# atakan-topaloglu/stable-virtual-camera

Hardware: AMD Instinct MI355X
Metric: denoising steps/sec, 1.3B Seva @ 21x576x576 views (higher is better)
Workload: dtype f16; 1 GPU; Seva 1.3B (1,263,968,004 params, random-init), one 21-view window per GPU, 576x576 px (latent 72x72), CFG batch 42, Euler-EDM step, MultiviewCFG(1.2) cfg 2.0; novel_views_per_sec = value x (T - 1 input view) / 50 steps per window; views=21, latent=72, windows=1

## Files before the change

stable-virtual-camera_amd/csrc/capi.hip:

```cpp
#include "seva_common.h"

#include <stdarg.h>
#include <stdio.h>
#include <stdlib.h>
#include <string.h>

#include <mutex>
#include <vector>

namespace {

thread_local char g_err[512] = "";

struct ProfRecord {
  int cls;
  double work, bytes;
  hipEvent_t e0, e1;
};
std::mutex g_prof_mu;
std::vector<ProfRecord> g_prof;
bool g_prof_on = false;

}

namespace {
struct KnobEntry {
  const char* name;
  const char* env;
  int SevaKnobs::*field;
};
const KnobEntry kKnobs[] = {
    {"gemm_chunks", "SEVA_GEMM_CHUNKS", &SevaKnobs::gemm_chunks}, {"gemm_dbg", "SEVA_GEMM_DBG", &SevaKnobs::gemm_dbg},
    {"gemm_stagger", "SEVA_GEMM_STAGGER", &SevaKnobs::gemm_stagger},
    {"gemm_bm", "SEVA_GEMM_BM", &SevaKnobs::gemm_bm}, {"gemm_bn", "SEVA_GEMM_BN", &SevaKnobs::gemm_bn},
    {"gemm_astat", "SEVA_GEMM_ASTAT", &SevaKnobs::gemm_astat}, {"attn_dbg", "SEVA_ATTN_DBG", &SevaKnobs::attn_dbg},
    {"attn_no_tr", "SEVA_ATTN_NO_TR", &SevaKnobs::attn_no_tr}, {"attn_two", "SEVA_ATTN_TWO", &SevaKnobs::attn_two},
    {"attn_split", "SEVA_ATTN_SPLIT", &SevaKnobs::attn_split},
    {"gn_min_iter", "SEVA_GN_MIN_ITER", &SevaKnobs::gn_min_iter},
    {"conv_win", "SEVA_CONV_WIN", &SevaKnobs::conv_win},
};
SevaKnobs knobs_from_env() {
  SevaKnobs k;
  for (const auto& e : kKnobs) {
    const char* v = getenv(e.env);
    k.*(e.field) = (v && v[0]) ? atoi(v) : -1;
  }
  return k;
}
}

SevaKnobs g_seva_knobs = knobs_from_env();

thread_local const char* g_seva_last_plan = "";

void seva_set_error(const char* fmt, ...) {
  va_list ap;
  va_start(ap, fmt);
  vsnprintf(g_err, sizeof(g_err), fmt, ap);
  va_end(ap);
}

int seva_check_launch(const char* what) {
  hipError_t e = hipGetLastError();
  if (e != hipSuccess) {
    seva_set_error("%s: launch failed: %s", what, hipGetErrorString(e));
    return SEVA_ERR_LAUNCH;
  }
  return SEVA_OK;
}

SevaProfScope::SevaProfScope(int cls_, double work_, hipStream_t stream_, double bytes_)
    : cls(cls_), work(work_), bytes(bytes_ < 0 ? work_ : bytes_), stream(stream_), e0(nullptr), e1(nullptr), on(g_prof_on) {
  if (!on) return;
  if (hipEventCreate(&e0) != hipSuccess || hipEventCreate(&e1) != hipSuccess) {
    on = false;
    return;
  }
  (void)hipEventRecord(e0, stream);
}

SevaProfScope::~SevaProfScope() {
  if (!on) return;
  (void)hipEventRecord(e1, stream);
  std::lock_guard<std::mutex> lk(g_prof_mu);
  g_prof.push_back({cls, work, bytes, e0, e1});
}

extern "C" {

const char* seva_last_error(void) { return g_err; }
const char* seva_last_plan(void) { return g_seva_last_plan; }
int seva_abi_version(void) { return 12; }
const char* seva_target_arch(void) { return "gfx950"; }

int seva_set_knob(const char* name, int value) {
  SEVA_REQUIRE(name != nullptr, "set_knob: null name");
  for (const auto& e : kKnobs)
    if (strcmp(e.name, name) == 0) {
      g_seva_knobs.*(e.field) = value;
      return SEVA_OK;
    }
  seva_set_error("set_knob: unknown knob '%s'", name);
  return SEVA_ERR_ARG;
}

int seva_get_knob(const char* name, int* value) {
  SEVA_REQUIRE(name != nullptr && value != nullptr, "get_knob: null argument");
  for (const auto& e : kKnobs)
    if (strcmp(e.name, name) == 0) {
      *value = g_seva_knobs.*(e.field);
      return SEVA_OK;
    }
  seva_set_error("get_knob: unknown knob '%s'", name);
  return SEVA_ERR_ARG;
}

int seva_graph_begin(seva_stream_t stream) {
  hipError_t e = hipStreamBeginCapture((hipStream_t)stream, hipStreamCaptureModeThreadLocal);
  if (e != hipSuccess) {
    seva_set_error("graph_begin: %s", hipGetErrorString(e));
    return SEVA_ERR_LAUNCH;
  }
  return SEVA_OK;
}

int seva_graph_end(seva_stream_t stream, void** graph_exec_out) {
  SEVA_REQUIRE(graph_exec_out != nullptr, "graph_end: null out");
  hipGraph_t graph = nullptr;
  hipError_t e = hipStreamEndCapture((hipStream_t)stream, &graph);
  if (e != hipSuccess || graph == nullptr) {
    seva_set_error("graph_end: %s", hipGetErrorString(e));
    return SEVA_ERR_LAUNCH;
  }
  hipGraphExec_t exec = nullptr;
  e = hipGraphInstantiate(&exec, graph, nullptr, nullptr, 0);
  (void)hipGraphDestroy(graph);
  if (e != hipSuccess) {
    seva_set_error("graph_instantiate: %s", hipGetErrorString(e));
    return SEVA_ERR_LAUNCH;
  }
  *graph_exec_out = (void*)exec;
  return SEVA_OK;
}

int seva_graph_launch(void* graph_exec, seva_stream_t stream) {
  SEVA_REQUIRE(graph_exec != nullptr, "graph_launch: null graph");
  hipError_t e = hipGraphLaunch((hipGraphExec_t)graph_exec, (hipStream_t)stream);
  if (e != hipSuccess) {
    seva_set_error("graph_launch: %s", hipGetErrorString(e));
    return SEVA_ERR_LAUNCH;
  }
  return SEVA_OK;
}

int seva_graph_destroy(void* graph_exec) {
  if (graph_exec) (void)hipGraphExecDestroy((hipGraphExec_t)graph_exec);
  return SEVA_OK;
}

int seva_prof_enable(int on) {
  std::lock_guard<std::mutex> lk(g_prof_mu);
  g_prof_on = on != 0;
  return SEVA_OK;
}

int seva_prof_collect(double* ms, int64_t* launches, double* work, double* bytes) {
  SEVA_REQUIRE(ms && launches && work && bytes, "prof_collect: null out");
  hipError_t e = hipDeviceSynchronize();
  if (e != hipSuccess) {
    seva_set_error("prof_collect: %s", hipGetErrorString(e));
    return SEVA_ERR_LAUNCH;
  }
  std::lock_guard<std::mutex> lk(g_prof_mu);
  for (int i = 0; i < SEVA_PROF_CLASSES; ++i) {
    ms[i] = 0.0;
    launches[i] = 0;
    work[i] = 0.0;
    bytes[i] = 0.0;
  }
  for (auto& r : g_prof) {
    float t = 0.f;
    if (hipEventElapsedTime(&t, r.e0, r.e1) == hipSuccess && r.cls >= 0 && r.cls < SEVA_PROF_CLASSES) {
      ms[r.cls] += t;
      launches[r.cls] += 1;
      work[r.cls] += r.work;
      bytes[r.cls] += r.bytes;
    }
    (void)hipEventDestroy(r.e0);
    (void)hipEventDestroy(r.e1);
  }
  g_prof.clear();
  return SEVA_OK;
}

}
```

stable-virtual-camera_amd/csrc/ff_fused.hip:

```cpp
#include "gemm_common.h"
#include "ff_fp8.h"

#include <atomic>

namespace {

struct FfArgs {
  const half_t* a;
  const half_t* w1;
  const float* b1;
  const half_t* w2;
  const float* b2;
  const float* residual;
  float* out_f32;
  half_t* out_f16;
  int64_t M, lda, ldr, ldo32, ldo16;
  int32_t tiles_m;
  const float* ln_x;
  const float* ln_gamma;
  const float* ln_beta;
  int64_t ldx;
  float ln_eps;
};

struct Ff8Args {
  FfArgs f;
  const uint8_t* w1_exp;
  const uint8_t* w2_exp;
};

template <int N>
__device__ __forceinline__ void ff_wait_vm() {
  asm volatile("s_waitcnt vmcnt(%0)" ::"n"(N) : "memory");
}

static __device__ __forceinline__ void glds16_sv(const void* sbase, unsigned voff, unsigned lds_wave_base) {
  unsigned keep;
  asm volatile(
      "s_mov_b32 %0, m0\n\ts_mov_b32 m0, %3\n\ts_nop 0\n\tglobal_load_lds_dwordx4 %1, %2\n\ts_mov_b32 m0, %0"
      : "=&s"(keep)
      : "v"(voff), "s"(sbase), "s"(lds_wave_base)
      : "memory");
}


template <int C>
__global__ __launch_bounds__(512, 2) void ff_fused8_kernel(FfArgs p) {
  constexpr int KS = C / 32, NK1 = C / 64, NJ2 = C / 16, NJH = NJ2 / 2, NCH = C / 16;
  constexpr int W1_BYTES = 128 * 128, W2_BYTES = C * 128;
  constexpr int W2_PASSES = C / 64;
  constexpr int W2_PER_KT = (W2_PASSES + NK1 - 1) / NK1;
  static_assert(NJ2 % 2 == 0, "output blocks split over the two waves of a row group");

  extern __shared__ __attribute__((aligned(16))) char smem[];
  constexpr int W1_RING = 3;
  char* const lds_w1 = smem;
  char* const lds_w2 = smem + W1_RING * W1_BYTES;
  float* const lds_b1 = (float*)(smem + W1_RING * W1_BYTES + 2 * W2_BYTES);
  char* const lds_x = smem + W1_RING * W1_BYTES + 2 * W2_BYTES + 8 * C * 4;
  const unsigned lds_base_u32 = __builtin_amdgcn_readfirstlane(lds_addr_u32(smem));

  const int lane = threadIdx.x & 63;
  const int wave = __builtin_amdgcn_readfirstlane(threadIdx.x >> 6);
  const int mr = wave & 3, h = wave >> 2;
  const int fr = lane & 15, fg = lane >> 4;
  const int sr = lane >> 3, sp = lane & 7;

  const int tm = xcd_remap(blockIdx.x, p.tiles_m);
  const int64_t m0 = (int64_t)tm * 128 + mr * 32;

  half8_t areg[2][KS];
  if (p.ln_x) {
#pragma unroll
    for (int i = 0; i < 2; ++i) {
      int64_t m = m0 + 16 * i + fr;
      if (m >= p.M) m = p.M - 1;
      const float* xr = p.ln_x + m * p.ldx + 8 * fg;
      f32x4 v[KS][2];
#pragma unroll
      for (int ks = 0; ks < KS; ++ks) {
        v[ks][0] = first_read(*(const f32x4*)(xr + 32 * ks));
        v[ks][1] = first_read(*(const f32x4*)(xr + 32 * ks + 4));
      }
      float sum = 0.f;
#pragma unroll
      for (int ks = 0; ks < KS; ++ks)
#pragma unroll
        for (int e = 0; e < 2; ++e) sum += v[ks][e][0] + v[ks][e][1] + v[ks][e][2] + v[ks][e][3];
      sum += __shfl_xor(sum, 16, 64);
      asm volatile("" : "+v"(sum));
      sum += __shfl_xor(sum, 32, 64);
      asm volatile("" : "+v"(sum));
      const float mean = sum / (float)C;
      float ss = 0.f;
#pragma unroll
      for (int ks = 0; ks < KS; ++ks)
#pragma unroll
        for (int e = 0; e < 2; ++e)
#pragma unroll
          for (int r = 0; r < 4; ++r) {
            const float dlt = v[ks][e][r] - mean;
            ss += dlt * dlt;
          }
      ss += __shfl_xor(ss, 16, 64);
      asm volatile("" : "+v"(ss));
      ss += __shfl_xor(ss, 32, 64);
      asm volatile("" : "+v"(ss));
      const float rstd = rsqrtf(ss / (float)C + p.ln_eps);
#pragma unroll
      for (int ks = 0; ks < KS; ++ks) {
        half_t y[8];
#pragma unroll
        for (int e = 0; e < 2; ++e) {
          const f32x4 g4 = first_read(*(const f32x4*)(p.ln_gamma + 32 * ks + 8 * fg + 4 * e));
          const f32x4 b4 = first_read(*(const f32x4*)(p.ln_beta + 32 * ks + 8 * fg + 4 * e));
#pragma unroll
          for (int r = 0; r < 4; ++r) y[4 * e + r] = (half_t)((v[ks][e][r] - mean) * rstd * g4[r] + b4[r]);
        }
        areg[i][ks] = half8_t{y[0], y[1], y[2], y[3], y[4], y[5], y[6], y[7]};
      }
    }
  } else {
#pragma unroll
    for (int i = 0; i < 2; ++i) {
      int64_t m = m0 + 16 * i + fr;
      if (m >= p.M) m = p.M - 1;
      const half_t* ap = p.a + m * p.lda + 8 * fg;
#pragma unroll
      for (int ks = 0; ks < KS; ++ks) areg[i][ks] = *(const half8_t*)(ap + 32 * ks);
    }
  }
  f32x4 acc2[2][NJH];
#pragma unroll
  for (int i = 0; i < 2; ++i) {
    int64_t m = m0 + 16 * i + fr;
    if (m >= p.M) m = p.M - 1;
#pragma unroll
    for (int jj = 0; jj < NJH; ++jj)
      acc2[i][jj] = p.residual ? *(const f32x4*)(p.residual + m * p.ldr + 16 * (h * NJH + jj) + 4 * fg) : f32x4{0.f, 0.f, 0.f, 0.f};
  }
  for (int i = threadIdx.x; i < 2 * C; i += 512) *(f32x4*)(lds_b1 + 4 * i) = *(const f32x4*)(p.b1 + 4 * i);
#pragma unroll
  for (int i = 0; i < 2; ++i) {
#pragma unroll
    for (int ks = 0; ks < KS; ++ks) asm volatile("" : "+v"(areg[i][ks]));
#pragma unroll
    for (int jj = 0; jj < NJH; ++jj) asm volatile("" : "+v"(acc2[i][jj]));
  }

  auto w1_key = [](int row) { return ((row >> 1) & 1) | (((row >> 3) & 3) << 1); };
  const half_t* w1_src[2];
#pragma unroll
  for (int i = 0; i < 2; ++i) {
    const int row = wave * 16 + 8 * i + sr;
    w1_src[i] = p.w1 + (int64_t)row * C + (sp ^ w1_key(row)) * 8;
  }
  const half_t* w2_src[2];
#pragma unroll
  for (int i = 0; i < 2; ++i) {
    const int row = wave * (C / 8) + 8 * i + sr;
    w2_src[i] = p.w2 + (int64_t)row * (4 * C) + (sp ^ ((row >> 1) & 7)) * 8;
  }
  auto stage_w1 = [&](int buf, int hc, int kt) {
    const unsigned dst = lds_base_u32 + buf * W1_BYTES + wave * 16 * 128;
    const int64_t off = (int64_t)hc * 128 * C + kt * 64;
#pragma unroll
    for (int i = 0; i < 2; ++i) glds16_raw(w1_src[i] + off, dst + i * 1024);
  };
  auto stage_w2_part = [&](int buf, int hc, int part) {
    const unsigned dst = lds_base_u32 + W1_RING * W1_BYTES + buf * W2_BYTES + wave * (C / 8) * 128;
#pragma unroll
    for (int u = 0; u < W2_PER_KT; ++u) {
      const int i = part * W2_PER_KT + u;
      if (i < W2_PASSES) glds16_raw(w2_src[i & 1] + (int64_t)(i >> 1) * 16 * (4 * C) + hc * 64, dst + i * 1024);
    }
  };
  auto barrier_raw = [&]() {
    asm volatile("s_waitcnt lgkmcnt(0)" ::: "memory");
    __builtin_amdgcn_s_barrier();
    asm volatile("" ::: "memory");
  };

  int w1_off[2], w2_off[2];
#pragma unroll
  for (int s = 0; s < 2; ++s) {
    const int rb = 64 * h + 8 * (fr >> 2) + (fr & 3);
    w1_off[s] = rb * 128 + (((4 * s + fg) ^ w1_key(rb)) << 4);
    const int r2 = 16 * (h * NJH) + fr;
    w2_off[s] = r2 * 128 + (((4 * s + fg) ^ ((r2 >> 1) & 7)) << 4);
  }
  char* const x_mine = lds_x + ((mr * 2 + h) * 2) * 1024 + lane * 16;
  const char* const x_q0 = lds_x + (mr * 2 * 2) * 1024 + lane * 16;

  constexpr int NTILES = NCH * NK1;
  auto stage_w1_seq = [&](int g) { stage_w1(g % W1_RING, g / NK1, g % NK1); };
  auto wait_all_but = [&](int n) {
    if (n >= 3) ff_wait_vm<3>();
    else if (n == 2) ff_wait_vm<2>();
    else if (n == 1) ff_wait_vm<1>();
    else ff_wait_vm<0>();
  };
  __syncthreads();
  stage_w1_seq(0);
#pragma unroll
  for (int part = 0; part < NK1; ++part) stage_w2_part(0, 0, part);
  if (NTILES > 1) stage_w1_seq(1);
  if (NTILES > 1) ff_wait_vm<2>();
  else ff_wait_vm<0>();
  barrier_raw();

  int g = 0;
  for (int hc = 0; hc < NCH; ++hc) {
    f32x4 acc1[2][4];
#pragma unroll
    for (int e = 0; e < 2; ++e) {
      const float* bp = lds_b1 + hc * 128 + 64 * h + 8 * fg + 4 * e;
      acc1[0][e] = acc1[1][e] = *(const f32x4*)bp;
      acc1[0][2 + e] = acc1[1][2 + e] = *(const f32x4*)(bp + 32);
    }
#pragma unroll
    for (int kt = 0; kt < NK1; ++kt) {
      int issued = 0;
      if (g + 2 < NTILES) {
        stage_w1_seq(g + 2);
        issued += 2;
      }
      if (hc + 1 < NCH && kt * W2_PER_KT < W2_PASSES) {
        stage_w2_part((hc + 1) & 1, hc + 1, kt);
        issued += (kt + 1) * W2_PER_KT <= W2_PASSES ? W2_PER_KT : W2_PASSES - kt * W2_PER_KT;
      }
      const char* const tb = lds_w1 + (g % W1_RING) * W1_BYTES;
      half8_t bfr[2][4];
#pragma unroll
      for (int s = 0; s < 2; ++s)
#pragma unroll
        for (int j = 0; j < 4; ++j) bfr[s][j] = *(const half8_t*)(tb + w1_off[s] + (32 * (j >> 1) + 4 * (j & 1)) * 128);
#pragma unroll
      for (int s = 0; s < 2; ++s)
#pragma unroll
        for (int i = 0; i < 2; ++i)
#pragma unroll
          for (int j = 0; j < 4; ++j)
            acc1[i][j] = __builtin_amdgcn_mfma_f32_16x16x32_f16(bfr[s][j], areg[i][2 * kt + s], acc1[i][j], 0, 0, 0);
      wait_all_but(issued);
      barrier_raw();
      ++g;
    }
#pragma unroll
    for (int i = 0; i < 2; ++i) {
      const f32x4 o0 = geglu4(acc1[i][0], acc1[i][2]);
      const f32x4 o1 = geglu4(acc1[i][1], acc1[i][3]);
      *(half8_t*)(x_mine + i * 1024) = half8_t{(half_t)o0[0], (half_t)o0[1], (half_t)o0[2], (half_t)o0[3],
                                               (half_t)o1[0], (half_t)o1[1], (half_t)o1[2], (half_t)o1[3]};
    }
    barrier_raw();
    half8_t hq[2][2];
#pragma unroll
    for (int q = 0; q < 2; ++q)
#pragma unroll
      for (int i = 0; i < 2; ++i) hq[q][i] = *(const half8_t*)(x_q0 + (q * 2 + i) * 1024);
    const char* const t2 = lds_w2 + (hc & 1) * W2_BYTES;
#pragma unroll
    for (int jj = 0; jj < NJH; ++jj) {
      const half8_t w0 = *(const half8_t*)(t2 + w2_off[0] + jj * (16 * 128));
      const half8_t w1f = *(const half8_t*)(t2 + w2_off[1] + jj * (16 * 128));
#pragma unroll
      for (int i = 0; i < 2; ++i) {
        acc2[i][jj] = __builtin_amdgcn_mfma_f32_16x16x32_f16(w0, hq[0][i], acc2[i][jj], 0, 0, 0);
        acc2[i][jj] = __builtin_amdgcn_mfma_f32_16x16x32_f16(w1f, hq[1][i], acc2[i][jj], 0, 0, 0);
      }
    }
    barrier_raw();
  }

#pragma unroll
  for (int i = 0; i < 2; ++i) {
    const int64_t m = m0 + 16 * i + fr;
    const bool ok = m < p.M;
#pragma unroll
    for (int jj = 0; jj < NJH; ++jj) {
      const int f = 16 * (h * NJH + jj) + 4 * fg;
      const f32x4 v = acc2[i][jj] + first_read(*(const f32x4*)(p.b2 + f));
      if (!ok) continue;
      if (p.out_f32) *(f32x4*)(p.out_f32 + m * p.ldo32 + f) = v;
      if (p.out_f16) {
        const half4_t hh = {(half_t)v[0], (half_t)v[1], (half_t)v[2], (half_t)v[3]};
        *(half4_t*)(p.out_f16 + m * p.ldo16 + f) = hh;
      }
    }
  }
}


template <int C>
int ff_launch8(const FfArgs& a, hipStream_t s) {
  constexpr int lds = 3 * 128 * 128 + 2 * C * 128 + 8 * C * 4 + 16 * 1024;
  static std::atomic<uint64_t> attr_devs{0};
  int dev = 0;
  (void)hipGetDevice(&dev);
  const uint64_t bit = 1ull << (dev & 63);
  if (!(attr_devs.load(std::memory_order_relaxed) & bit)) {
    (void)hipFuncSetAttribute((const void*)ff_fused8_kernel<C>, hipFuncAttributeMaxDynamicSharedMemorySize, lds);
    attr_devs.fetch_or(bit, std::memory_order_relaxed);
  }
  hipLaunchKernelGGL((ff_fused8_kernel<C>), dim3((unsigned)a.tiles_m), dim3(512), lds, s, a);
  return seva_check_launch("ff_fused8_kernel");
}


template <int C>
__global__ __launch_bounds__(512, 2) void ff_fused8_fp8_kernel(Ff8Args q) {
  const FfArgs& p = q.f;
  constexpr int KP = FF8_KP(C), NK1 = KP / 128, NU = C / 64;
  constexpr int NJ2 = C / 16, NJH = NJ2 / 2, NCH = C / 16, NP = NCH / 2, NSC2 = (NJH + 3) / 4;
  constexpr int W1_BYTES = 128 * 128, W2_BYTES = C * 128;
  constexpr int W2_PASSES = C / 64;
  constexpr int W2_PER_KT = (W2_PASSES + 2 * NK1 - 1) / (2 * NK1);
  static_assert(NJ2 % 2 == 0 && NCH % 2 == 0, "output blocks split over two waves; chunks taken in pairs");
  static_assert(2 + W2_PER_KT <= 3, "wait_all_but counts at most 3 loads per K-tile");
  typedef int v4i_t __attribute__((ext_vector_type(4)));

  extern __shared__ __attribute__((aligned(16))) char smem[];
  constexpr int W1_RING = 3;
  char* const lds_w1 = smem;
  char* const lds_w2 = smem + W1_RING * W1_BYTES;
  float* const lds_b1 = (float*)(smem + W1_RING * W1_BYTES + 2 * W2_BYTES);
  int* const lds_s1 = (int*)(smem + W1_RING * W1_BYTES + 2 * W2_BYTES + 8 * C * 4);
  char* const lds_x = smem + W1_RING * W1_BYTES + 2 * W2_BYTES + 8 * C * 4 + NCH * 32 * 4;
  const unsigned lds_base_u32 = __builtin_amdgcn_readfirstlane(lds_addr_u32(smem));

  const int lane = threadIdx.x & 63;
  const int wave = __builtin_amdgcn_readfirstlane(threadIdx.x >> 6);
  const int mr = wave & 3, h = wave >> 2;
  const int fr = lane & 15, fg = lane >> 4;
  const int sr = lane >> 3, sp = lane & 7;

  const int tm = xcd_remap(blockIdx.x, p.tiles_m);
  const int64_t m0 = (int64_t)tm * 128 + mr * 32;

  half8_t areg[2][2 * NK1];
  if (p.ln_x) {
#pragma unroll
    for (int i = 0; i < 2; ++i) {
      int64_t m = m0 + 16 * i + fr;
      if (m >= p.M) m = p.M - 1;
      const float* xr = p.ln_x + m * p.ldx + 16 * fg;
      f32x4 v[NU][4];
#pragma unroll
      for (int u = 0; u < NU; ++u)
#pragma unroll
        for (int e = 0; e < 4; ++e) v[u][e] = first_read(*(const f32x4*)(xr + 64 * u + 4 * e));
      float sum = 0.f;
#pragma unroll
      for (int u = 0; u < NU; ++u)
#pragma unroll
        for (int e = 0; e < 4; ++e) sum += v[u][e][0] + v[u][e][1] + v[u][e][2] + v[u][e][3];
      sum += __shfl_xor(sum, 16, 64);
      asm volatile("" : "+v"(sum));
      sum += __shfl_xor(sum, 32, 64);
      asm volatile("" : "+v"(sum));
      const float mean = sum / (float)C;
      float ss = 0.f;
#pragma unroll
      for (int u = 0; u < NU; ++u)
#pragma unroll
        for (int e = 0; e < 4; ++e)
#pragma unroll
          for (int r = 0; r < 4; ++r) {
            const float dlt = v[u][e][r] - mean;
            ss += dlt * dlt;
          }
      ss += __shfl_xor(ss, 16, 64);
      asm volatile("" : "+v"(ss));
      ss += __shfl_xor(ss, 32, 64);
      asm volatile("" : "+v"(ss));
      const float rstd = rsqrtf(ss / (float)C + p.ln_eps);
#pragma unroll
      for (int u = 0; u < 2 * NK1; ++u) {
        if (u >= NU) {
          areg[i][u] = half8_t{};
          continue;
        }
        v4i_t w;
#pragma unroll
        for (int e = 0; e < 4; ++e) {
          const f32x4 g4 = first_read(*(const f32x4*)(p.ln_gamma + 64 * u + 16 * fg + 4 * e));
          const f32x4 b4 = first_read(*(const f32x4*)(p.ln_beta + 64 * u + 16 * fg + 4 * e));
          float y[4];
#pragma unroll
          for (int r = 0; r < 4; ++r) y[r] = (v[u][e][r] - mean) * rstd * g4[r] + b4[r];
          w[e] = pack_fp8x4(y[0], y[1], y[2], y[3]);
        }
        areg[i][u] = __builtin_bit_cast(half8_t, w);
      }
    }
  } else {
#pragma unroll
    for (int i = 0; i < 2; ++i) {
      int64_t m = m0 + 16 * i + fr;
      if (m >= p.M) m = p.M - 1;
      const uint8_t* ap = (const uint8_t*)p.a + m * p.lda + 16 * fg;
#pragma unroll
      for (int u = 0; u < 2 * NK1; ++u) areg[i][u] = u < NU ? *(const half8_t*)(ap + 64 * u) : half8_t{};
    }
  }
  f32x4 acc2[2][NJH];
#pragma unroll
  for (int i = 0; i < 2; ++i)
#pragma unroll
    for (int jj = 0; jj < NJH; ++jj) acc2[i][jj] = f32x4{0.f, 0.f, 0.f, 0.f};
  for (int i = threadIdx.x; i < 2 * C; i += 512) *(f32x4*)(lds_b1 + 4 * i) = *(const f32x4*)(p.b1 + 4 * i);
  for (int idx = threadIdx.x; idx < NCH * 32; idx += 512) {
    const int hc = idx >> 5, hh = (idx >> 4) & 1, f = idx & 15;
    const int rb = hc * 128 + 64 * hh + 8 * (f >> 2) + (f & 3);
    lds_s1[idx] = (int)q.w1_exp[rb] | ((int)q.w1_exp[rb + 4] << 8) | ((int)q.w1_exp[rb + 32] << 16) | ((int)q.w1_exp[rb + 36] << 24);
  }
  int wsc2[NSC2];
#pragma unroll
  for (int w = 0; w < NSC2; ++w) wsc2[w] = 0;
#pragma unroll
  for (int jj = 0; jj < NJH; ++jj) wsc2[jj >> 2] |= (int)q.w2_exp[16 * (h * NJH + jj) + fr] << (8 * (jj & 3));
#pragma unroll
  for (int i = 0; i < 2; ++i) {
#pragma unroll
    for (int u = 0; u < NU; ++u) asm volatile("" : "+v"(areg[i][u]));
#pragma unroll
    for (int jj = 0; jj < NJH; ++jj) asm volatile("" : "+v"(acc2[i][jj]));
  }
#pragma unroll
  for (int w = 0; w < NSC2; ++w) asm volatile("" : "+v"(wsc2[w]));

  auto w1_key = [](int row) { return ((row >> 1) & 1) | (((row >> 3) & 3) << 1); };
  unsigned w1_voff[2];
#pragma unroll
  for (int i = 0; i < 2; ++i) {
    const int row = wave * 16 + 8 * i + sr;
    w1_voff[i] = (unsigned)(row * KP + (sp ^ w1_key(row)) * 16);
  }
  unsigned w2_voff[2];
#pragma unroll
  for (int i = 0; i < 2; ++i) {
    const int row = wave * (C / 8) + 8 * i + sr;
    w2_voff[i] = (unsigned)(row * (4 * C) + (sp ^ ((row >> 1) & 7)) * 16);
  }
  auto stage_w1 = [&](int buf, int hc, int kt) {
    const unsigned dst = lds_base_u32 + buf * W1_BYTES + wave * 16 * 128;
    const uint8_t* const base = (const uint8_t*)p.w1 + (int64_t)hc * 128 * KP + kt * 128;
#pragma unroll
    for (int i = 0; i < 2; ++i) glds16_sv(base, w1_voff[i], dst + i * 1024);
  };
  auto stage_w2_part = [&](int buf, int pp, int part) {
    const unsigned dst = lds_base_u32 + W1_RING * W1_BYTES + buf * W2_BYTES + wave * (C / 8) * 128;
#pragma unroll
    for (int u = 0; u < W2_PER_KT; ++u) {
      const int i = part * W2_PER_KT + u;
      if (i < W2_PASSES)
        glds16_sv((const uint8_t*)p.w2 + (int64_t)(i >> 1) * 16 * (4 * C) + pp * 128, w2_voff[i & 1], dst + i * 1024);
    }
  };
  auto barrier_raw = [&]() {
    asm volatile("s_waitcnt lgkmcnt(0)" ::: "memory");
    __builtin_amdgcn_s_barrier();
    asm volatile("" ::: "memory");
  };

  int w1_off[2], w2_off[2];
#pragma unroll
  for (int s = 0; s < 2; ++s) {
    const int rb = 64 * h + 8 * (fr >> 2) + (fr & 3);
    w1_off[s] = rb * 128 + (((4 * s + fg) ^ w1_key(rb)) << 4);
    const int r2 = 16 * (h * NJH) + fr;
    w2_off[s] = r2 * 128 + (((4 * s + fg) ^ ((r2 >> 1) & 7)) << 4);
  }
  char* const x_mine = lds_x + ((mr * 2 + h) * 2) * 1024 + lane * 16;
  const char* const x_q0 = lds_x + (mr * 2 * 2) * 1024 + lane * 16;

  constexpr int NTILES = NCH * NK1;
  auto stage_w1_seq = [&](int g) { stage_w1(g % W1_RING, g / NK1, g % NK1); };
  auto wait_all_but = [&](int n) {
    if (n >= 3) ff_wait_vm<3>();
    else if (n == 2) ff_wait_vm<2>();
    else if (n == 1) ff_wait_vm<1>();
    else ff_wait_vm<0>();
  };
  __syncthreads();
  stage_w1_seq(0);
#pragma unroll
  for (int part = 0; part < 2 * NK1; ++part) stage_w2_part(0, 0, part);
  stage_w1_seq(1);
  ff_wait_vm<2>();
  barrier_raw();

  int g = 0;
  for (int pp = 0; pp < NP; ++pp) {
    v4i_t hx[2];
#pragma unroll
    for (int c = 0; c < 2; ++c) {
      const int hc = 2 * pp + c;
      f32x4 acc1[2][4];
#pragma unroll
      for (int i = 0; i < 2; ++i)
#pragma unroll
        for (int j = 0; j < 4; ++j) acc1[i][j] = f32x4{0.f, 0.f, 0.f, 0.f};
      const int sc1 = lds_s1[hc * 32 + h * 16 + fr];
#pragma unroll
      for (int kt = 0; kt < NK1; ++kt) {
        int issued = 0;
        if (g + 2 < NTILES) {
          stage_w1_seq(g + 2);
          issued += 2;
        }
        const int kk = c * NK1 + kt;
        if (pp + 1 < NP && kk * W2_PER_KT < W2_PASSES) {
          stage_w2_part((pp + 1) & 1, pp + 1, kk);
          issued += (kk + 1) * W2_PER_KT <= W2_PASSES ? W2_PER_KT : W2_PASSES - kk * W2_PER_KT;
        }
        const char* const tb = lds_w1 + (g % W1_RING) * W1_BYTES;
#pragma unroll
        for (int jp = 0; jp < 2; ++jp) {
          half8_t bfr[2][2];
#pragma unroll
          for (int s = 0; s < 2; ++s)
#pragma unroll
            for (int e = 0; e < 2; ++e) bfr[s][e] = *(const half8_t*)(tb + w1_off[s] + (32 * jp + 4 * e) * 128);
#pragma unroll
          for (int i = 0; i < 2; ++i)
#pragma unroll
            for (int e = 0; e < 2; ++e)
              acc1[i][2 * jp + e] = mfma_f8(2 * jp + e, bfr[0][e], bfr[1][e], areg[i][2 * kt], areg[i][2 * kt + 1], acc1[i][2 * jp + e], sc1);
          if (jp == 0) __builtin_amdgcn_sched_barrier(0);
        }
#pragma unroll
        for (int i = 0; i < 2; ++i)
#pragma unroll
          for (int j = 0; j < 4; ++j) asm volatile("" : "+v"(acc1[i][j]));
        wait_all_but(issued);
        barrier_raw();
        ++g;
      }
      f32x4 bias[4];
#pragma unroll
      for (int e = 0; e < 2; ++e) {
        const float* bp = lds_b1 + hc * 128 + 64 * h + 8 * fg + 4 * e;
        bias[e] = first_read(*(const f32x4*)bp);
        bias[2 + e] = first_read(*(const f32x4*)(bp + 32));
      }
#pragma unroll
      for (int i = 0; i < 2; ++i) {
        const f32x4 o0 = geglu4(acc1[i][0] + bias[0], acc1[i][2] + bias[2]);
        const f32x4 o1 = geglu4(acc1[i][1] + bias[1], acc1[i][3] + bias[3]);
        hx[i][2 * c] = pack_fp8x4(o0[0], o0[1], o0[2], o0[3]);
        hx[i][2 * c + 1] = pack_fp8x4(o1[0], o1[1], o1[2], o1[3]);
      }
    }
#pragma unroll
    for (int i = 0; i < 2; ++i) *(v4i_t*)(x_mine + i * 1024) = hx[i];
    barrier_raw();
    half8_t hq[2][2];
#pragma unroll
    for (int qq = 0; qq < 2; ++qq)
#pragma unroll
      for (int i = 0; i < 2; ++i) hq[qq][i] = *(const half8_t*)(x_q0 + (qq * 2 + i) * 1024);
    const char* const t2 = lds_w2 + (pp & 1) * W2_BYTES;
#pragma unroll
    for (int jj = 0; jj < NJH; ++jj) {
      const half8_t w0 = *(const half8_t*)(t2 + w2_off[0] + jj * (16 * 128));
      const half8_t w1f = *(const half8_t*)(t2 + w2_off[1] + jj * (16 * 128));
#pragma unroll
      for (int i = 0; i < 2; ++i) acc2[i][jj] = mfma_f8(jj, w0, w1f, hq[0][i], hq[1][i], acc2[i][jj], wsc2[jj >> 2]);
    }
#pragma unroll
    for (int i = 0; i < 2; ++i)
#pragma unroll
      for (int jj = 0; jj < NJH; ++jj) asm volatile("" : "+v"(acc2[i][jj]));
    barrier_raw();
  }

#pragma unroll
  for (int i = 0; i < 2; ++i) {
    const int64_t m = m0 + 16 * i + fr;
    const bool ok = m < p.M;
#pragma unroll
    for (int jj = 0; jj < NJH; ++jj) {
      const int f = 16 * (h * NJH + jj) + 4 * fg;
      if (!ok) continue;
      f32x4 v = acc2[i][jj] + first_read(*(const f32x4*)(p.b2 + f));
      if (p.residual) v += first_read(*(const f32x4*)(p.residual + m * p.ldr + f));
      if (p.out_f32) *(f32x4*)(p.out_f32 + m * p.ldo32 + f) = v;
      if (p.out_f16) {
        const half4_t hh = {(half_t)v[0], (half_t)v[1], (half_t)v[2], (half_t)v[3]};
        *(half4_t*)(p.out_f16 + m * p.ldo16 + f) = hh;
      }
    }
  }
}

template <int C>
int ff_launch8_fp8(const Ff8Args& a, hipStream_t s) {
  constexpr int lds = 3 * 128 * 128 + 2 * C * 128 + 8 * C * 4 + (C / 16) * 32 * 4 + 16 * 1024;
  static_assert(lds <= 160 * 1024, "LDS budget of one workgroup per CU");
  static std::atomic<uint64_t> attr_devs{0};
  int dev = 0;
  (void)hipGetDevice(&dev);
  const uint64_t bit = 1ull << (dev & 63);
  if (!(attr_devs.load(std::memory_order_relaxed) & bit)) {
    (void)hipFuncSetAttribute((const void*)ff_fused8_fp8_kernel<C>, hipFuncAttributeMaxDynamicSharedMemorySize, lds);
    attr_devs.fetch_or(bit, std::memory_order_relaxed);
  }
// ... 84 lines not shown
```

stable-virtual-camera_amd/csrc/gemm_plan_dump.cpp:

```cpp
#include <stdio.h>
#include <stdlib.h>
#include <string.h>

#include <string>

#include "gemm_plan.h"

using namespace seva_plan;

static void print_gemm_cfg(const GemmCfg& c) {
  printf("\tbm=%d\tbn=%d\tmode=%d\tepi=%d\tdbgk=%d\tpaired=%d\tastat=%d\tfp8=%d\tsplitk=%d\tnw=%d\tsplit16=%d", c.bm, c.bn, c.mode, c.epi, c.dbgk,
         c.paired, c.astat, c.fp8, c.splitk, c.nw, c.split16);
}
static void print_win_cfg(const WinCfg& c) {
  printf("\tbm=%d\tbn=%d\tnw=%d\twcap=%d\tdbw=%d\tstats=%d\tup=%d\ttw=%d\tfp8=%d\to8=%d\ts2=%d\tph=%d", c.bm, c.bn, c.nw, c.wcap, c.dbw, c.stats,
         c.up, c.tw, c.fp8, c.o8, c.s2, c.ph);
}

static int print_tables() {
  for (int i = 0; i < kNumGemmKernels; ++i) {
    printf("table=gemm\trow=%d\tname=%s\thas_dbgk=%d", i, kGemmKernels[i].name, has_dbgk(kGemmKernels[i].cfg));
    print_gemm_cfg(kGemmKernels[i].cfg);
    printf("\n");
  }
  for (int i = 0; i < kNumWinKernels; ++i) {
    printf("table=win\trow=%d\tname=%s", i, kWinKernels[i].name);
    print_win_cfg(kWinKernels[i].cfg);
    printf("\n");
  }
  return 0;
}

int main() {
  static char line[4096];
  void* const set = (void*)(uintptr_t)64;
  while (fgets(line, sizeof line, stdin)) {
    if (strncmp(line, "tables", 6) == 0) {
      print_tables();
      continue;
    }
    seva_gemm_desc d;
    memset(&d, 0, sizeof d);
    SevaKnobs k;
    k.gemm_chunks = k.gemm_dbg = k.gemm_stagger = k.gemm_bm = k.gemm_bn = k.gemm_astat = -1;
    k.attn_dbg = k.attn_no_tr = k.attn_two = k.attn_split = k.gn_min_iter = k.conv_win = -1;
    Variant v = F16;
    bool any = false, bad = false;
    for (char* tok = strtok(line, " \t\r\n"); tok; tok = strtok(nullptr, " \t\r\n")) {
      char* eq = strchr(tok, '=');
      if (!eq) { bad = true; break; }
      *eq = 0;
      const std::string key = tok, val = eq + 1;
      const long long x = atoll(val.c_str());
      any = true;
      if (key == "v") v = val == "fp8" ? FP8 : val == "split_out" ? F16_SPLIT_OUT : F16;
      else if (key == "mode") d.mode = (int)x;
      else if (key == "epi") d.epilogue = (int)x;
      else if (key == "M") d.M = x;
      else if (key == "N") d.N = x;
      else if (key == "K") d.K = x;
      else if (key == "n") d.n = (int)x;
      else if (key == "ih") d.ih = (int)x;
      else if (key == "iw") d.iw = (int)x;
      else if (key == "cin") d.cin = (int)x;
      else if (key == "oh") d.oh = (int)x;
      else if (key == "ow") d.ow = (int)x;
      else if (key == "stride") d.stride = (int)x;
      else if (key == "up") d.upsample = (int)x;
      else if (key == "pad_br") d.pad_br_only = (int)x;
      else if (key == "rpg") d.rows_per_group = x;
      else if (key == "K2") d.K2 = x;
      else if (key == "bias") d.bias = x ? (const float*)set : nullptr;
      else if (key == "row_add") d.row_add = x ? (const float*)set : nullptr;
      else if (key == "residual") d.residual = x ? (const float*)set : nullptr;
      else if (key == "out_f32") d.out_f32 = x ? (float*)set : nullptr;
      else if (key == "out_f16") d.out_f16 = x ? set : nullptr;
      else if (key == "out_f8") d.out_f8 = x ? set : nullptr;
      else if (key == "w_exp") d.w_exp = x ? set : nullptr;
      else if (key == "ch_stats") d.ch_stats = x ? (float*)set : nullptr;
      else if (key == "splitk_ws") d.splitk_ws = x ? (float*)set : nullptr;
      else if (key == "a2") d.a2 = x ? set : nullptr;
      else if (key == "gemm_bm") k.gemm_bm = (int)x;
      else if (key == "gemm_bn") k.gemm_bn = (int)x;
      else if (key == "gemm_astat") k.gemm_astat = (int)x;
      else if (key == "gemm_chunks") k.gemm_chunks = (int)x;
      else if (key == "gemm_dbg") k.gemm_dbg = (int)x;
      else if (key == "gemm_stagger") k.gemm_stagger = (int)x;
      else if (key == "conv_win") k.conv_win = (int)x;
      else { bad = true; break; }
    }
    if (!any) continue;
    if (bad) {
      printf("kernel=bad_input\n");
      continue;
    }
    d.a = set;
    d.w = set;
    const Plan p = plan(d, k, v);
    const WinPlan& w = p.window;
    static const char* const declined[] = {"none", "phases", "fp8_stride2", "fp8_window_only"};
    if (p.declined != DECLINED_NONE) {
      printf("kernel=error\tdeclined=%s", declined[p.declined]);
    } else if (p.kernel == GEMM_KERNEL) {
      const int row = find_row(p.gemm);
      printf("kernel=gemm\trow=%d\tname=%s", row, row >= 0 ? kGemmKernels[row].name : "NONE");
      print_gemm_cfg(p.gemm);
      printf("\ttiles_m=%d\ttiles_n=%d\tchunks=%d\tgrid=%lld\tdbg=%d\tstagger=%d\tsk_tiles=%lld\tsk_bn=%d", p.tiles_m, p.tiles_n, p.n_chunks,
             (long long)p.grid, p.dbg, p.stagger, (long long)p.sk_tiles, p.sk_bn);
    } else {
      const WinCfg& c = w.cand[w.win];
      const int row = find_row(c);
      printf("kernel=window\trow=%d\tname=%s", row, row >= 0 ? kWinKernels[row].name : "NONE");
      print_win_cfg(c);
      printf("\tlinear=%d\tn_lin=%d\tranges=%d\tn_full=%d\tfull=%d/%d/%d\ttail=%d/%d/%d\ttiles_n=%d", w.linear, w.geom.n_lin, w.n_ranges(), w.n_full,
             w.full.n, w.full.tpi, w.full.tiles_m, w.tail.n, w.tail.tpi, w.tail.tiles_m, w.geom.tiles_n);
      printf("\tWp=%d\tSp=%d\thw=%d\tow=%d\tmul=%u/%u/%u/%u", w.geom.Wp, w.geom.Sp, w.geom.hw, w.geom.ow, w.geom.mul_hw, w.geom.mul_iw, w.geom.mul_sp,
             w.geom.mul_wp);
    }
    printf("\twin=%d\tcands=", w.win);
    for (int i = 0; i < w.n_cand; ++i) {
      const int row = find_row(w.cand[i]);
      printf("%s%s", i ? ";" : "", row >= 0 ? kWinKernels[row].name : "NONE");
    }
    printf("\n");
  }
  return 0;
}
```

stable-virtual-camera_amd/csrc/seva_knobs.h:

```cpp
#pragma once

struct SevaKnobs {
  int gemm_chunks, gemm_dbg, gemm_stagger, gemm_bm, gemm_bn, gemm_astat;
  int attn_dbg, attn_no_tr, attn_two, attn_split;
  int gn_min_iter;
  int conv_win;
};
extern SevaKnobs g_seva_knobs;
```

Before: 11.04 denoising steps/s.

## Make fused FF kernel persistent with cross-tile weight prefetch and LDS-resident biases

Converts the fused feed-forward kernel into a persistent grid sized from an occupancy query, with each workgroup looping over M tiles. While the current tile's epilogue runs, the next tile's first W1/W2 weight tiles are already being staged. Biases b1 and b2 are loaded into LDS once per workgroup instead of once per tile, and kernel arguments are read through the kernarg pointer to ease scalar register pressure. The intent is to remove per-tile launch and prologue latency and overlap it with compute. The cost is a larger LDS footprint, a new ff_grid knob, and a risk of load imbalance when the tile count does not divide evenly across the grid.

Result: no change. 11.03 denoising steps/s (-0.1%).

```diff
diff --git a/stable-virtual-camera_amd/csrc/capi.hip b/stable-virtual-camera_amd/csrc/capi.hip
--- a/stable-virtual-camera_amd/csrc/capi.hip
+++ b/stable-virtual-camera_amd/csrc/capi.hip
@@ -37,6 +37,7 @@
     {"attn_no_tr", "SEVA_ATTN_NO_TR", &SevaKnobs::attn_no_tr}, {"attn_two", "SEVA_ATTN_TWO", &SevaKnobs::attn_two},
     {"attn_split", "SEVA_ATTN_SPLIT", &SevaKnobs::attn_split},
     {"gn_min_iter", "SEVA_GN_MIN_ITER", &SevaKnobs::gn_min_iter},
+    {"ff_grid", "SEVA_FF_GRID", &SevaKnobs::ff_grid},
     {"conv_win", "SEVA_CONV_WIN", &SevaKnobs::conv_win},
 };
 SevaKnobs knobs_from_env() {
diff --git a/stable-virtual-camera_amd/csrc/ff_fused.hip b/stable-virtual-camera_amd/csrc/ff_fused.hip
--- a/stable-virtual-camera_amd/csrc/ff_fused.hip
+++ b/stable-virtual-camera_amd/csrc/ff_fused.hip
@@ -43,6 +43,12 @@
       : "memory");
 }
 
+typedef const __attribute__((address_space(4))) FfArgs* ff_kargs_t;
+static __device__ __forceinline__ ff_kargs_t ff_kargs() {
+  ff_kargs_t q = (ff_kargs_t)__builtin_amdgcn_kernarg_segment_ptr();
+  asm volatile("" : "+s"(q));
+  return q;
+}
 
 template <int C>
 __global__ __launch_bounds__(512, 2) void ff_fused8_kernel(FfArgs p) {
@@ -58,30 +64,106 @@
   char* const lds_w2 = smem + W1_RING * W1_BYTES;
   float* const lds_b1 = (float*)(smem + W1_RING * W1_BYTES + 2 * W2_BYTES);
   char* const lds_x = smem + W1_RING * W1_BYTES + 2 * W2_BYTES + 8 * C * 4;
+  constexpr int B2_OFF = W1_RING * W1_BYTES + 2 * W2_BYTES + 8 * C * 4 + 16 * 1024;
+  const float* const lds_b2 = (const float*)(smem + B2_OFF);
   const unsigned lds_base_u32 = __builtin_amdgcn_readfirstlane(lds_addr_u32(smem));
 
   const int lane = threadIdx.x & 63;
   const int wave = __builtin_amdgcn_readfirstlane(threadIdx.x >> 6);
   const int mr = wave & 3, h = wave >> 2;
-  const int fr = lane & 15, fg = lane >> 4;
-  const int sr = lane >> 3, sp = lane & 7;
-
-  const int tm = xcd_remap(blockIdx.x, p.tiles_m);
+  for (int i = threadIdx.x; i < 2 * C; i += 512) *(f32x4*)(lds_b1 + 4 * i) = *(const f32x4*)(p.b1 + 4 * i);
+  for (int i = threadIdx.x; i < C / 4; i += 512) *(f32x4*)(smem + B2_OFF + 16 * i) = *(const f32x4*)(p.b2 + 4 * i);
+
+  auto w1_key = [](int row) { return ((row >> 1) & 1) | (((row >> 3) & 3) << 1); };
+  const half_t* w1_src[2];
+  const half_t* w2_src[2];
+  auto set_src = [&](int ln) {
+    const int sr = ln >> 3, sp = ln & 7;
+#pragma unroll
+    for (int i = 0; i < 2; ++i) {
+      const int row = wave * 16 + 8 * i + sr;
+      w1_src[i] = p.w1 + (int64_t)row * C + (sp ^ w1_key(row)) * 8;
+    }
+#pragma unroll
+    for (int i = 0; i < 2; ++i) {
+      const int row = wave * (C / 8) + 8 * i + sr;
+      w2_src[i] = p.w2 + (int64_t)row * (4 * C) + (sp ^ ((row >> 1) & 7)) * 8;
+    }
+  };
+  set_src(lane);
+  auto stage_w1 = [&](int buf, int hc, int kt) {
+    const unsigned dst = lds_base_u32 + buf * W1_BYTES + wave * 16 * 128;
+    const int64_t off = (int64_t)hc * 128 * C + kt * 64;
+#pragma unroll
+    for (int i = 0; i < 2; ++i) glds16_raw(w1_src[i] + off, dst + i * 1024);
+  };
+  auto stage_w2_part = [&](int buf, int hc, int part) {
+    const unsigned dst = lds_base_u32 + W1_RING * W1_BYTES + buf * W2_BYTES + wave * (C / 8) * 128;
+#pragma unroll
+    for (int u = 0; u < W2_PER_KT; ++u) {
+      const int i = part * W2_PER_KT + u;
+      if (i < W2_PASSES) glds16_raw(w2_src[i & 1] + (int64_t)(i >> 1) * 16 * (4 * C) + hc * 64, dst + i * 1024);
+    }
+  };
+  auto barrier_raw = [&]() {
+    asm volatile("s_waitcnt lgkmcnt(0)" ::: "memory");
+    __builtin_amdgcn_s_barrier();
+    asm volatile("" ::: "memory");
+  };
+
+  constexpr int NTILES = NCH * NK1;
+  auto stage_w1_seq = [&](int g) { stage_w1(g % W1_RING, g / NK1, g % NK1); };
+  auto stage_head = [&]() {
+    const half_t *s1a = w1_src[0], *s1b = w1_src[1], *s2a = w2_src[0], *s2b = w2_src[1];
+    unsigned lb = lds_base_u32;
+    asm volatile("" : "+v"(s1a), "+v"(s1b), "+v"(s2a), "+v"(s2b), "+s"(lb));
+    const unsigned d1 = lb + wave * 16 * 128, d2 = lb + W1_RING * W1_BYTES + wave * (C / 8) * 128;
+    glds16_raw(s1a, d1);
+    glds16_raw(s1b, d1 + 1024);
+#pragma unroll
+    for (int i = 0; i < W2_PASSES; ++i) glds16_raw(((i & 1) ? s2b : s2a) + (int64_t)(i >> 1) * 16 * (4 * C), d2 + i * 1024);
+    if (NTILES > 1) {
+      constexpr int64_t off = (int64_t)(1 / NK1) * 128 * C + (1 % NK1) * 64;
+      glds16_raw(s1a + off, d1 + W1_BYTES);
+      glds16_raw(s1b + off, d1 + W1_BYTES + 1024);
+    }
+  };
+  auto wait_all_but = [&](int n) {
+    if (n >= 3) ff_wait_vm<3>();
+    else if (n == 2) ff_wait_vm<2>();
+    else if (n == 1) ff_wait_vm<1>();
+    else ff_wait_vm<0>();
+  };
+  static_assert(2 + W2_PER_KT <= 3, "wait_all_but counts at most 3 loads per K-tile");
+
+  const int grid = (int)gridDim.x;
+  stage_head();
+  for (int vb = (int)blockIdx.x; vb < p.tiles_m; vb += grid) {
+  const int tm = xcd_remap(vb, p.tiles_m);
   const int64_t m0 = (int64_t)tm * 128 + mr * 32;
-
+  const bool more = vb + grid < p.tiles_m;
+  int lane_t = lane;
+  asm volatile("" : "+v"(lane_t));
+  const int fr = lane_t & 15, fg = lane_t >> 4;
+
+  const ff_kargs_t ph = ff_kargs();
   half8_t areg[2][KS];
-  if (p.ln_x) {
+  if (ph->ln_x) {
+    f32x4 vv[2][KS][2];
 #pragma unroll
     for (int i = 0; i < 2; ++i) {
       int64_t m = m0 + 16 * i + fr;
-      if (m >= p.M) m = p.M - 1;
-      const float* xr = p.ln_x + m * p.ldx + 8 * fg;
-      f32x4 v[KS][2];
+      if (m >= ph->M) m = ph->M - 1;
+      const float* xr = ph->ln_x + m * ph->ldx + 8 * fg;
 #pragma unroll
       for (int ks = 0; ks < KS; ++ks) {
-        v[ks][0] = first_read(*(const f32x4*)(xr + 32 * ks));
-        v[ks][1] = first_read(*(const f32x4*)(xr + 32 * ks + 4));
-      }
+        vv[i][ks][0] = first_read(*(const f32x4*)(xr + 32 * ks));
+        vv[i][ks][1] = first_read(*(const f32x4*)(xr + 32 * ks + 4));
+      }
+    }
+#pragma unroll
+    for (int i = 0; i < 2; ++i) {
+      f32x4(&v)[KS][2] = vv[i];
       float sum = 0.f;
 #pragma unroll
       for (int ks = 0; ks < KS; ++ks)
@@ -106,26 +188,27 @@
       asm volatile("" : "+v"(ss));
       ss += __shfl_xor(ss, 32, 64);
       asm volatile("" : "+v"(ss));
-      const float rstd = rsqrtf(ss / (float)C + p.ln_eps);
+      const float rstd = rsqrtf(ss / (float)C + ph->ln_eps);
 #pragma unroll
       for (int ks = 0; ks < KS; ++ks) {
         half_t y[8];
 #pragma unroll
         for (int e = 0; e < 2; ++e) {
-          const f32x4 g4 = first_read(*(const f32x4*)(p.ln_gamma + 32 * ks + 8 * fg + 4 * e));
-          const f32x4 b4 = first_read(*(const f32x4*)(p.ln_beta + 32 * ks + 8 * fg + 4 * e));
+          const f32x4 g4 = first_read(*(const f32x4*)(ph->ln_gamma + 32 * ks + 8 * fg + 4 * e));
+          const f32x4 b4 = first_read(*(const f32x4*)(ph->ln_beta + 32 * ks + 8 * fg + 4 * e));
 #pragma unroll
           for (int r = 0; r < 4; ++r) y[4 * e + r] = (half_t)((v[ks][e][r] - mean) * rstd * g4[r] + b4[r]);
         }
         areg[i][ks] = half8_t{y[0], y[1], y[2], y[3], y[4], y[5], y[6], y[7]};
       }
+      if (i == 0) __builtin_amdgcn_sched_barrier(0);
     }
   } else {
 #pragma unroll
     for (int i = 0; i < 2; ++i) {
       int64_t m = m0 + 16 * i + fr;
-      if (m >= p.M) m = p.M - 1;
-      const half_t* ap = p.a + m * p.lda + 8 * fg;
+      if (m >= ph->M) m = ph->M - 1;
+      const half_t* ap = ph->a + m * ph->lda + 8 * fg;
 #pragma unroll
       for (int ks = 0; ks < KS; ++ks) areg[i][ks] = *(const half8_t*)(ap + 32 * ks);
     }
@@ -134,12 +217,11 @@
 #pragma unroll
   for (int i = 0; i < 2; ++i) {
     int64_t m = m0 + 16 * i + fr;
-    if (m >= p.M) m = p.M - 1;
+    if (m >= ph->M) m = ph->M - 1;
 #pragma unroll
     for (int jj = 0; jj < NJH; ++jj)
-      acc2[i][jj] = p.residual ? *(const f32x4*)(p.residual + m * p.ldr + 16 * (h * NJH + jj) + 4 * fg) : f32x4{0.f, 0.f, 0.f, 0.f};
-  }
-  for (int i = threadIdx.x; i < 2 * C; i += 512) *(f32x4*)(lds_b1 + 4 * i) = *(const f32x4*)(p.b1 + 4 * i);
+      acc2[i][jj] = ph->residual ? *(const f32x4*)(ph->residual + m * ph->ldr + 16 * (h * NJH + jj) + 4 * fg) : f32x4{0.f, 0.f, 0.f, 0.f};
+  }
 #pragma unroll
   for (int i = 0; i < 2; ++i) {
 #pragma unroll
@@ -148,65 +230,22 @@
     for (int jj = 0; jj < NJH; ++jj) asm volatile("" : "+v"(acc2[i][jj]));
   }
 
-  auto w1_key = [](int row) { return ((row >> 1) & 1) | (((row >> 3) & 3) << 1); };
-  const half_t* w1_src[2];
-#pragma unroll
-  for (int i = 0; i < 2; ++i) {
-    const int row = wave * 16 + 8 * i + sr;
-    w1_src[i] = p.w1 + (int64_t)row * C + (sp ^ w1_key(row)) * 8;
-  }
-  const half_t* w2_src[2];
-#pragma unroll
-  for (int i = 0; i < 2; ++i) {
-    const int row = wave * (C / 8) + 8 * i + sr;
-    w2_src[i] = p.w2 + (int64_t)row * (4 * C) + (sp ^ ((row >> 1) & 7)) * 8;
-  }
-  auto stage_w1 = [&](int buf, int hc, int kt) {
-    const unsigned dst = lds_base_u32 + buf * W1_BYTES + wave * 16 * 128;
-    const int64_t off = (int64_t)hc * 128 * C + kt * 64;
-#pragma unroll
-    for (int i = 0; i < 2; ++i) glds16_raw(w1_src[i] + off, dst + i * 1024);
-  };
-  auto stage_w2_part = [&](int buf, int hc, int part) {
-    const unsigned dst = lds_base_u32 + W1_RING * W1_BYTES + buf * W2_BYTES + wave * (C / 8) * 128;
-#pragma unroll
-    for (int u = 0; u < W2_PER_KT; ++u) {
-      const int i = part * W2_PER_KT + u;
-      if (i < W2_PASSES) glds16_raw(w2_src[i & 1] + (int64_t)(i >> 1) * 16 * (4 * C) + hc * 64, dst + i * 1024);
-    }
-  };
-  auto barrier_raw = [&]() {
-    asm volatile("s_waitcnt lgkmcnt(0)" ::: "memory");
-    __builtin_amdgcn_s_barrier();
-    asm volatile("" ::: "memory");
-  };
-
+  int lane_c = lane;
+  asm volatile("" : "+v"(lane_c));
+  set_src(lane_c);
+  const int fr_c = lane_c & 15, fg_c = lane_c >> 4;
   int w1_off[2], w2_off[2];
 #pragma unroll
   for (int s = 0; s < 2; ++s) {
-    const int rb = 64 * h + 8 * (fr >> 2) + (fr & 3);
-    w1_off[s] = rb * 128 + (((4 * s + fg) ^ w1_key(rb)) << 4);
-    const int r2 = 16 * (h * NJH) + fr;
-    w2_off[s] = r2 * 128 + (((4 * s + fg) ^ ((r2 >> 1) & 7)) << 4);
-  }
-  char* const x_mine = lds_x + ((mr * 2 + h) * 2) * 1024 + lane * 16;
-  const char* const x_q0 = lds_x + (mr * 2 * 2) * 1024 + lane * 16;
-
-  constexpr int NTILES = NCH * NK1;
-  auto stage_w1_seq = [&](int g) { stage_w1(g % W1_RING, g / NK1, g % NK1); };
-  auto wait_all_but = [&](int n) {
-    if (n >= 3) ff_wait_vm<3>();
-    else if (n == 2) ff_wait_vm<2>();
-    else if (n == 1) ff_wait_vm<1>();
-    else ff_wait_vm<0>();
-  };
-  __syncthreads();
-  stage_w1_seq(0);
-#pragma unroll
-  for (int part = 0; part < NK1; ++part) stage_w2_part(0, 0, part);
-  if (NTILES > 1) stage_w1_seq(1);
-  if (NTILES > 1) ff_wait_vm<2>();
-  else ff_wait_vm<0>();
+    const int rb = 64 * h + 8 * (fr_c >> 2) + (fr_c & 3);
+    w1_off[s] = rb * 128 + (((4 * s + fg_c) ^ w1_key(rb)) << 4);
+    const int r2 = 16 * (h * NJH) + fr_c;
+    w2_off[s] = r2 * 128 + (((4 * s + fg_c) ^ ((r2 >> 1) & 7)) << 4);
+  }
+  char* const x_mine = lds_x + ((mr * 2 + h) * 2) * 1024 + lane_c * 16;
+  const char* const x_q0 = lds_x + (mr * 2 * 2) * 1024 + lane_c * 16;
+
+  ff_wait_vm<0>();
   barrier_raw();
 
   int g = 0;
@@ -214,7 +253,7 @@
     f32x4 acc1[2][4];
 #pragma unroll
     for (int e = 0; e < 2; ++e) {
-      const float* bp = lds_b1 + hc * 128 + 64 * h + 8 * fg + 4 * e;
+      const float* bp = lds_b1 + hc * 128 + 64 * h + 8 * fg_c + 4 * e;
       acc1[0][e] = acc1[1][e] = *(const f32x4*)bp;
       acc1[0][2 + e] = acc1[1][2 + e] = *(const f32x4*)(bp + 32);
     }
@@ -273,37 +312,59 @@
     barrier_raw();
   }
 
+  if (more) stage_head();
+
+  const ff_kargs_t pe = ff_kargs();
+  int lane_e = lane;
+  asm volatile("" : "+v"(lane_e));
+  const int fr_e = lane_e & 15, fg_e = lane_e >> 4;
 #pragma unroll
   for (int i = 0; i < 2; ++i) {
-    const int64_t m = m0 + 16 * i + fr;
-    const bool ok = m < p.M;
+    const int64_t m = m0 + 16 * i + fr_e;
+    const bool ok = m < pe->M;
 #pragma unroll
     for (int jj = 0; jj < NJH; ++jj) {
-      const int f = 16 * (h * NJH + jj) + 4 * fg;
-      const f32x4 v = acc2[i][jj] + first_read(*(const f32x4*)(p.b2 + f));
+      const int f = 16 * (h * NJH + jj) + 4 * fg_e;
+      const f32x4 v = acc2[i][jj] + first_read(*(const f32x4*)(lds_b2 + f));
       if (!ok) continue;
-      if (p.out_f32) *(f32x4*)(p.out_f32 + m * p.ldo32 + f) = v;
-      if (p.out_f16) {
+      if (pe->out_f32) *(f32x4*)(pe->out_f32 + m * pe->ldo32 + f) = v;
+      if (pe->out_f16) {
         const half4_t hh = {(half_t)v[0], (half_t)v[1], (half_t)v[2], (half_t)v[3]};
-        *(half4_t*)(p.out_f16 + m * p.ldo16 + f) = hh;
-      }
-    }
-  }
-}
-
+        *(half4_t*)(pe->out_f16 + m * pe->ldo16 + f) = hh;
+      }
+    }
+  }
+  }
+}
+
+
+template <int C>
+int ff_resident8(int lds) {
+  static std::atomic<int> resident[64];
+  int dev = 0;
+  (void)hipGetDevice(&dev);
+  int r = resident[dev & 63].load(std::memory_order_relaxed);
+  if (r > 0) return r;
+  int per_cu = 0, cus = 0;
+  if (hipFuncSetAttribute((const void*)ff_fused8_kernel<C>, hipFuncAttributeMaxDynamicSharedMemorySize, lds) != hipSuccess) return 0;
+  if (hipOccupancyMaxActiveBlocksPerMultiprocessor(&per_cu, ff_fused8_kernel<C>, 512, (size_t)lds) != hipSuccess) return 0;
+  if (hipDeviceGetAttribute(&cus, hipDeviceAttributeMultiprocessorCount, dev) != hipSuccess) return 0;
+  if (per_cu < 1 || cus < 1) return 0;
+  r = per_cu * cus;
+  resident[dev & 63].store(r, std::memory_order_relaxed);
+  return r;
+}
 
 template <int C>
 int ff_launch8(const FfArgs& a, hipStream_t s) {
-  constexpr int lds = 3 * 128 * 128 + 2 * C * 128 + 8 * C * 4 + 16 * 1024;
-  static std::atomic<uint64_t> attr_devs{0};
-  int dev = 0;
-  (void)hipGetDevice(&dev);
-  const uint64_t bit = 1ull << (dev & 63);
-  if (!(attr_devs.load(std::memory_order_relaxed) & bit)) {
-    (void)hipFuncSetAttribute((const void*)ff_fused8_kernel<C>, hipFuncAttributeMaxDynamicSharedMemorySize, lds);
-    attr_devs.fetch_or(bit, std::memory_order_relaxed);
-  }
-  hipLaunchKernelGGL((ff_fused8_kernel<C>), dim3((unsigned)a.tiles_m), dim3(512), lds, s, a);
+  constexpr int lds = 3 * 128 * 128 + 2 * C * 128 + 8 * C * 4 + 16 * 1024 + C * 4;
+  static_assert(lds <= 160 * 1024, "LDS budget of one workgroup per CU");
+  const int resident = ff_resident8<C>(lds);
+  SEVA_REQUIRE(resident > 0, "ff_fused: occupancy query of ff_fused8_kernel<%d> failed", C);
+  int grid = a.tiles_m < resident ? a.tiles_m : resident;
+  if (g_seva_knobs.ff_grid > 0 && g_seva_knobs.ff_grid < grid) grid = g_seva_knobs.ff_grid;
+  if (grid < a.tiles_m && grid >= 8) grid &= ~7;
+  hipLaunchKernelGGL((ff_fused8_kernel<C>), dim3((unsigned)grid), dim3(512), lds, s, a);
   return seva_check_launch("ff_fused8_kernel");
 }
 
diff --git a/stable-virtual-camera_amd/csrc/gemm_plan_dump.cpp b/stable-virtual-camera_amd/csrc/gemm_plan_dump.cpp
--- a/stable-virtual-camera_amd/csrc/gemm_plan_dump.cpp
+++ b/stable-virtual-camera_amd/csrc/gemm_plan_dump.cpp
@@ -43,7 +43,7 @@
     memset(&d, 0, sizeof d);
     SevaKnobs k;
     k.gemm_chunks = k.gemm_dbg = k.gemm_stagger = k.gemm_bm = k.gemm_bn = k.gemm_astat = -1;
-    k.attn_dbg = k.attn_no_tr = k.attn_two = k.attn_split = k.gn_min_iter = k.conv_win = -1;
+    k.attn_dbg = k.attn_no_tr = k.attn_two = k.attn_split = k.gn_min_iter = k.ff_grid = k.conv_win = -1;
     Variant v = F16;
     bool any = false, bad = false;
     for (char* tok = strtok(line, " \t\r\n"); tok; tok = strtok(nullptr, " \t\r\n")) {
diff --git a/stable-virtual-camera_amd/csrc/seva_knobs.h b/stable-virtual-camera_amd/csrc/seva_knobs.h
--- a/stable-virtual-camera_amd/csrc/seva_knobs.h
+++ b/stable-virtual-camera_amd/csrc/seva_knobs.h
@@ -4,6 +4,7 @@
   int gemm_chunks, gemm_dbg, gemm_stagger, gemm_bm, gemm_bn, gemm_astat;
   int attn_dbg, attn_no_tr, attn_two, attn_split;
   int gn_min_iter;
+  int ff_grid;
   int conv_win;
 };
 extern SevaKnobs g_seva_knobs;
```
